# diwakar-vsingh/EKF-SLAM

Hardware: NVIDIA B200
Metric: filter-steps/s at N=100 features, batch 4096 filters (higher is better)
Workload: dtype f64

## Files before the change

### ekf-slam_b200/csrc/abi.cu

```cuda
#include <cmath>
#include <cstdio>
#include <cstdlib>
#include <cstring>
#include <climits>
#include <string>
#include <vector>

#include "common.cuh"

static thread_local std::string g_err;
extern "C" { static void step_graph_destroy(ekfslam_ctx* c); }

static int fail(int code, const std::string& msg) {
    g_err = msg;
    return code;
}

#define CK(call)                                                                              \
    do {                                                                                      \
        cudaError_t _e = (call);                                                              \
        if (_e != cudaSuccess)                                                                \
            return fail(EKFSLAM_ERR_CUDA, std::string(#call) + ": " + cudaGetErrorName(_e) + \
                                              " (" + cudaGetErrorString(_e) + ")");           \
    } while (0)

#define NEED_CTX(c)                                                     \
    do {                                                                \
        if (!(c)) return fail(EKFSLAM_ERR_INVALID, "null context");     \
        CK(cudaSetDevice((c)->device));                                 \
    } while (0)

struct KTimer {
    struct Rec { cudaEvent_t a, b; int slot; };
    std::vector<Rec> pending;
    std::vector<cudaEvent_t> pool;
    double ms[KT_COUNT];
    long long count[KT_COUNT];
    cudaEvent_t cur[KT_COUNT];
};

static cudaEvent_t kt_event(KTimer* t) {
    if (!t->pool.empty()) { cudaEvent_t e = t->pool.back(); t->pool.pop_back(); return e; }
    cudaEvent_t e = nullptr;
    if (cudaEventCreate(&e) != cudaSuccess) { cudaGetLastError(); return nullptr; }
    return e;
}

void kt_begin(ekfslam_ctx* c, int slot) {
    KTimer* t = c->timer;
    t->cur[slot] = kt_event(t);
    if (t->cur[slot]) cudaEventRecord(t->cur[slot], c->stream);
}

static void kt_drain_completed(KTimer* t) {
    size_t done = 0;
    while (done < t->pending.size() && cudaEventQuery(t->pending[done].b) == cudaSuccess) {
        KTimer::Rec& r = t->pending[done];
        float ms = 0.f;
        if (cudaEventElapsedTime(&ms, r.a, r.b) == cudaSuccess) { t->ms[r.slot] += ms; t->count[r.slot]++; }
        t->pool.push_back(r.a);
        t->pool.push_back(r.b);
        ++done;
    }
    cudaGetLastError();
    if (done) t->pending.erase(t->pending.begin(), t->pending.begin() + done);
}

void kt_end(ekfslam_ctx* c, int slot) {
    KTimer* t = c->timer;
    KTimer::Rec r;
    r.a = t->cur[slot]; r.b = r.a ? kt_event(t) : nullptr; r.slot = slot;
    if (!r.a || !r.b) { if (r.a) t->pool.push_back(r.a); return; }
    cudaEventRecord(r.b, c->stream);
    t->pending.push_back(r);
    if (t->pending.size() > 1024) kt_drain_completed(t);
}

static void kt_collect(ekfslam_ctx* c) {
    KTimer* t = c->timer;
    if (!t) return;
    for (auto& r : t->pending) {
        float ms = 0.f;
        if (cudaEventElapsedTime(&ms, r.a, r.b) == cudaSuccess) { t->ms[r.slot] += ms; t->count[r.slot]++; }
        t->pool.push_back(r.a);
        t->pool.push_back(r.b);
    }
    t->pending.clear();
}

static const char* KT_NAMES[KT_COUNT] = {"k_begin_frame", "k_predict", "k_features", "k_hp", "k_innov", "k_ransac",
                                         "k_upd_S", "k_chol", "k_w", "k_downdate_hi", "k_downdate", "k_symmetrize",
                                         "k_add_features", "k_wfix", "k_w_hi", "k_chol_hi", "k_upd_S_hi",
                                         "k_hp_rescue", "k_world", "k_eval", "k_cam_update", "k_downdate_cam"};

template <typename T>
static cudaError_t dalloc(T** p, size_t count, int64_t* total) {
    const size_t bytes = count * sizeof(T);
    cudaError_t e = cudaMalloc((void**)p, bytes ? bytes : 1);
    if (e == cudaSuccess) {
        *total += (int64_t)bytes;
        e = cudaMemset(*p, 0, bytes ? bytes : 1);
    }
    return e;
}

extern "C" {
// ... 104 lines not shown
    DA(v.S, Bz * v.N * 4);
    DA(v.z, Bz * v.N * 2);
    DA(v.zc, Bz * v.N * 2);
    DA(v.ftype, Bz * v.N);
    DA(v.flags, Bz * v.N);
    DA(v.mflags, Bz * v.N);
    DA(v.foff, Bz * v.N);
    DA(v.nstate, Bz);
    DA(v.nfeat, Bz);
    DA(v.counters, Bz * v.N * 2);
    DA(v.tag, Bz * v.N);
    DA(c->mm_del, Bz * v.N);
    DA(c->mm_quota, Bz);
    DA(c->det_n, Bz);
    DA(v.sel, Bz * v.N);
    DA(v.ksel, Bz);
    DA(v.stats, Bz);
    DA(v.nhyp_tab, (size_t)(v.N + 1) * (v.N + 2) / 2);
#undef DA
    ekfslam_camera cam;
    ekfslam_default_camera(&cam);
    set_devcam(c, &cam);
    ekfslam_default_params(&c->prm);
    std::vector<int32_t> tab;
    build_nhyp_table(tab, v.N, c->prm.p_spurious_free);
    cudaError_t e = cudaMemcpy(v.nhyp_tab, tab.data(), tab.size() * sizeof(int32_t), cudaMemcpyHostToDevice);
    if (e == cudaSuccess) e = cudaStreamCreateWithFlags(&c->own_stream, cudaStreamNonBlocking);
    if (e == cudaSuccess) e = cudaStreamCreateWithFlags(&c->copy_stream, cudaStreamNonBlocking);
    if (e == cudaSuccess) e = cudaStreamCreateWithFlags(&c->aux_stream, cudaStreamNonBlocking);
    if (e == cudaSuccess) e = cudaStreamCreateWithFlags(&c->aux2_stream, cudaStreamNonBlocking);
    if (e == cudaSuccess) e = cudaEventCreateWithFlags(&c->ev_join2, cudaEventDisableTiming);
    if (e == cudaSuccess) e = cudaEventCreateWithFlags(&c->ev_fork, cudaEventDisableTiming);
    if (e == cudaSuccess) e = cudaEventCreateWithFlags(&c->ev_join, cudaEventDisableTiming);
    if (e == cudaSuccess) e = cudaMallocHost((void**)&c->kmax_host, sizeof(int32_t));
    if (e == cudaSuccess) e = cudaEventCreateWithFlags(&c->ev_in, cudaEventDisableTiming);
    if (e == cudaSuccess) e = cudaEventCreateWithFlags(&c->ev_out, cudaEventDisableTiming);
    if (e == cudaSuccess) e = cudaEventCreateWithFlags(&c->ev_main, cudaEventDisableTiming);
    if (e != cudaSuccess) {
        ekfslam_destroy(c);
        return fail(EKFSLAM_ERR_CUDA, std::string("context init: ") + cudaGetErrorString(e));
    }
    c->stream = c->own_stream;
    cudaDeviceGetAttribute(&c->sm_count, cudaDevAttrMultiProcessorCount, device);
    if (c->sm_count <= 0) c->sm_count = 148;
    *out = c;
    return EKFSLAM_OK;
}

int ekfslam_destroy(ekfslam_ctx* c) {
    if (!c) return EKFSLAM_OK;
    cudaSetDevice(c->device);
    if (c->own_zc) { c->v.zc = c->own_zc; c->v.mflags = c->own_mflags; c->v.u = c->own_u; c->own_zc = nullptr; }
    DevView& v = c->v;
    void* ptrs[] = {v.x, v.xp, v.P, v.G, v.W, v.Sb, v.Li, v.yv, v.jn, v.jnt, v.ktot, v.kmaxdev, v.cv, v.h, v.Hc, v.S, v.z, v.zc, v.u, v.ftype,
                    v.flags, v.mflags, v.foff, v.nstate, v.nfeat, v.counters, v.tag, v.sel, v.ksel, v.stats, v.nhyp_tab,
                    c->mm_del, c->mm_quota, c->det_n, c->det_uv, c->det_tag, c->world_points, c->world_poses,
                    c->ev.rec, c->ev.tot, c->ev.ferr, c->ev.fnees, c->ev.mp, c->ev.mc,
                    c->cu.H, c->cu.z, c->cu.R, c->cu.on, c->cu.nis, c->cu.status};
    for (void* p : ptrs)
        if (p) cudaFree(p);
    if (c->timer) {
        cudaStreamSynchronize(c->stream);
        kt_collect(c);
        for (cudaEvent_t e : c->timer->pool) cudaEventDestroy(e);
        delete c->timer;
        c->timer = nullptr;
    }
    step_graph_destroy(c);
    if (c->own_stream) cudaStreamDestroy(c->own_stream);
    if (c->copy_stream) cudaStreamDestroy(c->copy_stream);
    if (c->aux_stream) cudaStreamDestroy(c->aux_stream);
    if (c->aux2_stream) cudaStreamDestroy(c->aux2_stream);
    if (c->ev_join2) cudaEventDestroy(c->ev_join2);
    if (c->ev_fork) cudaEventDestroy(c->ev_fork);
    if (c->ev_join) cudaEventDestroy(c->ev_join);
    if (c->ev_in) cudaEventDestroy(c->ev_in);
    if (c->ev_out) cudaEventDestroy(c->ev_out);
    if (c->ev_main) cudaEventDestroy(c->ev_main);
    if (c->pin) cudaFree(c->pin);
    if (c->kmax_host) cudaFreeHost(c->kmax_host);
    delete c;
    return EKFSLAM_OK;
}

int ekfslam_set_stream(ekfslam_ctx* c, void* s) {
    NEED_CTX(c);
    c->stream = s ? (cudaStream_t)s : c->own_stream;
    return EKFSLAM_OK;
}

int ekfslam_set_camera(ekfslam_ctx* c, const ekfslam_camera* cam) {
    NEED_CTX(c);
    if (!cam) return fail(EKFSLAM_ERR_INVALID, "cam is null");
    if (!(cam->dx > 0) || !(cam->dy > 0) || cam->nRows <= 0 || cam->nCols <= 0)
        return fail(EKFSLAM_ERR_INVALID, "camera: dx, dy, nRows, nCols must be positive");
    set_devcam(c, cam);
    return EKFSLAM_OK;
}

int ekfslam_set_params(ekfslam_ctx* c, const ekfslam_params* p) {
    NEED_CTX(c);
    if (!p) return fail(EKFSLAM_ERR_INVALID, "params is null");
    if (p->max_hyp <= 0 || p->fixed_hyp < 0 || !(p->p_spurious_free > 0 && p->p_spurious_free < 1))
        return fail(EKFSLAM_ERR_INVALID, "params: max_hyp > 0, fixed_hyp >= 0, 0 < p_spurious_free < 1");
    const bool retab = p->p_spurious_free != c->prm.p_spurious_free;
    c->prm = *p;
    if (retab) {
        std::vector<int32_t> tab;
// ... 314 lines not shown
    launch_innov(c, mode);
    LAUNCHED();
    return EKFSLAM_OK;
}

int ekfslam_gate(ekfslam_ctx* c) {
    NEED_CTX(c);
    return gate_mode(c, 1);
}

int ekfslam_apply_matches(ekfslam_ctx* c) {
    NEED_CTX(c);
    return gate_mode(c, 2);
}

int ekfslam_ransac(ekfslam_ctx* c) {
    NEED_CTX(c);
    if (c->v.n_u <= 0) return fail(EKFSLAM_ERR_STATE, "ransac: no uniform stream uploaded (ekfslam_upload_uniforms)");
    launch_ransac(c);
    LAUNCHED();
    return EKFSLAM_OK;
}

int ekfslam_update_masked(ekfslam_ctx* c, int mask, int which_prior) {
    NEED_CTX(c);
    if (!(mask & 0xff)) return fail(EKFSLAM_ERR_INVALID, "empty mask");
    launch_update(c, mask, which_prior ? 1 : 0);
    LAUNCHED();
    return EKFSLAM_OK;
}

int ekfslam_update_li(ekfslam_ctx* c) {
    NEED_CTX(c);
    launch_hp(c, EKFSLAM_F_HAS_H | EKFSLAM_F_LI, 0);
    return ekfslam_update_masked(c, EKFSLAM_F_LI, 1);
}

int ekfslam_update_iterated(ekfslam_ctx* c, int mask, int which_prior, int n_iter) {
    NEED_CTX(c);
    if (!(mask & 0xff)) return fail(EKFSLAM_ERR_INVALID, "empty mask");
    if (n_iter < 1 || n_iter > 64) return fail(EKFSLAM_ERR_INVALID, "n_iter must be in [1, 64]");
    DevView& v = c->v;
    const size_t xbytes = sizeof(double) * (size_t)v.B * v.ld;
    if (which_prior) CK(cudaMemcpyAsync(v.x, v.xp, xbytes, cudaMemcpyDeviceToDevice, c->stream));
    else CK(cudaMemcpyAsync(v.xp, v.x, xbytes, cudaMemcpyDeviceToDevice, c->stream));
    for (int j = 0; j < n_iter; ++j) {
        launch_features(c, 0, 3);
        launch_hp(c, mask & 0xff, 0);
        launch_update(c, mask, 1, 1 | (j + 1 < n_iter ? 2 : 0));
    }
    LAUNCHED();
    return EKFSLAM_OK;
}

int ekfslam_rescue(ekfslam_ctx* c) {
    NEED_CTX(c);
    launch_features(c, 0, 3);
    launch_innov_gather(c, 3);
    launch_hp(c, EKFSLAM_F_HAS_H | EKFSLAM_F_HI, 0, KT_HP_RESCUE);
    LAUNCHED();
    return EKFSLAM_OK;
}

int ekfslam_update_hi(ekfslam_ctx* c) { return ekfslam_update_masked(c, EKFSLAM_F_HI, 0); }

int ekfslam_step(ekfslam_ctx* c, int reset, int match_mode) {
    NEED_CTX(c);
    if (match_mode < 0 || match_mode > 2) return fail(EKFSLAM_ERR_INVALID, "match_mode must be 0, 1 or 2");
    if (c->v.n_u <= 0) return fail(EKFSLAM_ERR_STATE, "step: no uniform stream uploaded");
    if (reset) launch_begin_frame(c);
    launch_predict(c);
    launch_features(c, 1, 3);
    launch_innov_gather(c, 0);
    if (c->wait_inputs) { cudaStreamWaitEvent(c->stream, c->ev_in, 0); c->wait_inputs = 0; }
    if (match_mode) launch_innov(c, match_mode);
    launch_ransac(c);
    {
        if (c->prm.fixed_hyp <= 0) launch_hp(c, EKFSLAM_F_HAS_H | EKFSLAM_F_LI, 0);
        launch_update(c, EKFSLAM_F_LI, 1);
        launch_features(c, 0, 3);
        launch_innov_gather(c, 3);
        launch_hp(c, EKFSLAM_F_HAS_H | EKFSLAM_F_HI, 0, KT_HP_RESCUE);
        launch_update(c, EKFSLAM_F_HI, 0);
    }
    LAUNCHED();
    return EKFSLAM_OK;
}

struct StepGraph {
    cudaGraphExec_t exec;
    DevView v; ekfslam_params prm; DevCam cam;
    int reset, match_mode;
    int64_t launches;
};

static void step_graph_destroy(ekfslam_ctx* c) {
    StepGraph* g = (StepGraph*)c->step_graph;
    if (g) { if (g->exec) cudaGraphExecDestroy(g->exec); delete g; c->step_graph = nullptr; }
}

int ekfslam_step_graph(ekfslam_ctx* c, int reset, int match_mode) {
    NEED_CTX(c);
    DevView& v = c->v;
    if (c->timer || chol_lockstep(v) || c->wait_inputs || c->arm_out) return ekfslam_step(c, reset, match_mode);
    if (match_mode < 0 || match_mode > 2) return fail(EKFSLAM_ERR_INVALID, "match_mode must be 0, 1 or 2");
    if (v.n_u <= 0) return fail(EKFSLAM_ERR_STATE, "step: no uniform stream uploaded");
    StepGraph* g = (StepGraph*)c->step_graph;
    if (g && (memcmp(&g->v, &v, sizeof(DevView)) || memcmp(&g->prm, &c->prm, sizeof(ekfslam_params)) ||
              memcmp(&g->cam, &c->cam, sizeof(DevCam)) || g->reset != reset || g->match_mode != match_mode)) {
        step_graph_destroy(c);
        g = nullptr;
    }
    if (!g) {
        g = new (std::nothrow) StepGraph();
        if (!g) return fail(EKFSLAM_ERR_NOMEM, "host allocation failed");
        memset(g, 0, sizeof(*g));
// ... 455 lines not shown
```

### ekf-slam_b200/csrc/common.cuh

```cuda
#pragma once
#include <cuda_runtime.h>
#include <stdint.h>
#include <mutex>
#include "../../include/ekfslam.h"

#define EKF_XV 13
#define EKF_HC 13
#define EKF_HSTRIDE 26

struct DevCam {
    double k1, k2, Cx, Cy, f, dx, dy;
    double fku, fkv;
    double nRows, nCols;
};

struct DevView {
    int B, N, nmax, ld;
    int kmax;
    int n_u;
    double* x;
    double* xp;
    double* P;
    double* G;
    double* W;
// ... 49 lines not shown
    ekfslam_eval* rec;
    ekfslam_eval* tot;
    double* ferr;
    double* fnees;
    double* mp;
    double* mc;
};

struct DevCamUpd {
    double* H;
    double* z;
    double* R;
    uint8_t* on;
    double* nis;
    int32_t* status;
    int m, b0, nb;
    double gate;
};

struct ekfslam_ctx {
    int device;
    KTimer* timer;
    DevView v;
    DevCam cam;
    ekfslam_params prm;
    cudaStream_t own_stream;
    cudaStream_t stream;
    int64_t bytes;
    int64_t launches;
    int stage;
    cudaStream_t copy_stream;
    cudaStream_t aux_stream, aux2_stream;
    cudaEvent_t ev_fork, ev_join, ev_join2;
    cudaEvent_t ev_in, ev_out, ev_main;
    int wait_inputs;
    int arm_out;
    void* pin;
    size_t pin_bytes;
    int u_cap;
    void* step_graph;
    int sm_count;
    int32_t* kmax_host;
    DevWorld world;
    double* world_points; double* world_poses;
    double* det_uv; int32_t* det_tag; int32_t* det_n; int det_K;
    uint8_t* mm_del; int32_t* mm_quota;
    double* own_zc; uint8_t* own_mflags; double* own_u; int own_n_u;
    DevEval ev;
    DevCamUpd cu;
};

#define EKF_WPAD 68
__host__ __device__ __forceinline__ size_t w_at(int wrows, int t, int c) {
    return ((size_t)(c >> 6) * wrows + t) * EKF_WPAD + (c & 63);
}

__device__ __forceinline__ void w_fold_jt(double* w, const double* Jt) {
    const double w3 = w[0], w4 = w[1], w5 = w[2], w6 = w[3];
#pragma unroll
    for (int i = 0; i < 4; ++i) w[i] = w3 * Jt[i * 4 + 0] + w4 * Jt[i * 4 + 1] + w5 * Jt[i * 4 + 2] + w6 * Jt[i * 4 + 3];
}

#define EKF_TRI(nic, s) (((nic) * ((nic) + 1)) / 2 + (s))

inline bool chol_lockstep(const DevView& v) { return v.B < 128 && v.kmax >= 256; }

inline std::mutex& ekf_attr_mutex() { static std::mutex m; return m; }

void kt_begin(ekfslam_ctx* c, int slot);
void kt_end(ekfslam_ctx* c, int slot);
struct KScope {
    ekfslam_ctx* c; int slot;
    KScope(ekfslam_ctx* c_, int s_) : c(c_), slot(s_) { if (c->timer) kt_begin(c, slot); }
    ~KScope() { if (c->timer) kt_end(c, slot); c->launches++; }
};

#define ENSURE_DYN_SMEM(func, bytes, dev)                                                                    \
    do {                                                                                                     \
        static size_t _hw[64];                                                                               \
        const size_t _b = (size_t)(bytes);                                                                   \
        const int _d = (dev) & 63;                                                                           \
        if (_b > 48 * 1024) {                                                                                \
            std::lock_guard<std::mutex> _g(ekf_attr_mutex());    \
            if (_b > _hw[_d]) {                                                                              \
                cudaFuncSetAttribute(func, cudaFuncAttributeMaxDynamicSharedMemorySize, (int)_b);            \
                _hw[_d] = _b;                                                                                \
            }                                                                                                \
        }                                                                                                    \
    } while (0)

void launch_begin_frame(ekfslam_ctx* c);
void launch_predict(ekfslam_ctx* c);
void launch_features(ekfslam_ctx* c, int which, int parts);
void launch_hp(ekfslam_ctx* c, int need, int forbid, int slot = KT_HP);
void launch_innov_gather(ekfslam_ctx* c, int mode);
void launch_innov(ekfslam_ctx* c, int mode);
void launch_symmetrize(ekfslam_ctx* c, int b0, int nb);
void launch_ransac(ekfslam_ctx* c);
void launch_update(ekfslam_ctx* c, int mask, int which_prior, int flags = 0);
void launch_downdate(ekfslam_ctx* c, int slot);
void launch_chol_blocked64(ekfslam_ctx* c, int kact);
void launch_reset_filters(ekfslam_ctx* c, int b0, int nb, const double* d_xv, const double* d_Pxv);
void launch_id2cart(ekfslam_ctx* c, double threshold, int force_index, int32_t* d_conv);
void launch_delete_features(ekfslam_ctx* c, int b0, int nb, const uint8_t* d_del);
void launch_add_features(ekfslam_ctx* c, int b0, int nb, const double* d_uvd, int uvd_stride, const uint8_t* d_add,
                         const int32_t* d_quota, int j, const int32_t* d_tag, int tag_stride,
                         double std_pxl, double rho0, double std_rho);
void launch_world_candidates(ekfslam_ctx* c, int t);
void launch_world_detect(ekfslam_ctx* c, int t);
void launch_world_uniforms(ekfslam_ctx* c, int t);
void launch_mm_plan(ekfslam_ctx* c, int min_features);
void launch_eval(ekfslam_ctx* c, int mode, int t, int b0, int nb);
void launch_cam_update(ekfslam_ctx* c, int which);
```

### ekf-slam_b200/csrc/k_model.cu

```cuda
#include <cstdlib>
#include "model.cuh"
#include "tc_common.cuh"

__global__ void k_begin_frame(DevView v) {
    const int t = blockIdx.x * blockDim.x + threadIdx.x;
    if (t >= v.B * v.N) return;
    const int b = t / v.N, i = t - b * v.N;
    if (i >= v.nfeat[b]) return;
    const uint8_t f = v.flags[t];
    if (f & EKFSLAM_F_HAS_H) v.counters[2 * t] += 1;
    if (f & (EKFSLAM_F_LI | EKFSLAM_F_HI)) v.counters[2 * t + 1] += 1;
    v.flags[t] = f & EKFSLAM_F_CAND;
}

void launch_begin_frame(ekfslam_ctx* c) {
    const int tot = c->v.B * c->v.N;
    KScope ks(c, KT_BEGIN_FRAME);
    k_begin_frame<<<(tot + 255) / 256, 256, 0, c->stream>>>(c->v);
}

__global__ void __launch_bounds__(256, 3) k_predict(DevView v, ekfslam_params prm) {
    const int b = blockIdx.x;
    const int n = v.nstate[b];
    const int ld = v.ld;
// ... 280 lines not shown
            for (int r = 0; r < 7; ++r) {
                g0.x += Hs[r] * pc[r].x; g0.y += Hs[r] * pc[r].y;
                g1.x += Hs[EKF_HC + r] * pc[r].x; g1.y += Hs[EKF_HC + r] * pc[r].y;
            }
            const int off = sOff[s];
            const int w = sW[s];
            const double* Pr = P + (size_t)off * ld + c0;
            if (w == 6) {
                double2 pf[6];
#pragma unroll
                for (int r = 0; r < 6; ++r) pf[r] = *reinterpret_cast<const double2*>(Pr + (size_t)r * ld);
#pragma unroll
                for (int r = 0; r < 6; ++r) {
                    g0.x += Hs[7 + r] * pf[r].x; g0.y += Hs[7 + r] * pf[r].y;
                    g1.x += Hs[EKF_HC + 7 + r] * pf[r].x; g1.y += Hs[EKF_HC + 7 + r] * pf[r].y;
                }
            } else {
                double2 pf[3];
#pragma unroll
                for (int r = 0; r < 3; ++r) pf[r] = *reinterpret_cast<const double2*>(Pr + (size_t)r * ld);
#pragma unroll
                for (int r = 0; r < 3; ++r) {
                    g0.x += Hs[7 + r] * pf[r].x; g0.y += Hs[7 + r] * pf[r].y;
                    g1.x += Hs[EKF_HC + 7 + r] * pf[r].x; g1.y += Hs[EKF_HC + 7 + r] * pf[r].y;
                }
            }
            const int i = sIdx[s];
            *reinterpret_cast<double2*>(G + (size_t)(2 * i) * ld + c0) = g0;
            *reinterpret_cast<double2*>(G + (size_t)(2 * i + 1) * ld + c0) = g1;
        }
    }
}

void launch_hp(ekfslam_ctx* c, int need, int forbid, int slot) {
    const int colchunks = (c->v.nmax + 255) / 256;
    const long long base = (long long)colchunks * c->v.B;
    const long long want = 4LL * c->sm_count;
    int fch = HP_CHUNK;
    while (fch > 8 && base * ((c->v.N + fch - 1) / fch) < want) fch >>= 1;
    int fz = (c->v.N + fch - 1) / fch;
    if (base >= want) fz = 1;
    else if (base * fz > want) fz = (int)((want + base - 1) / base);
    dim3 grid(colchunks, c->v.B, fz);
    KScope ks(c, slot);
    k_hp<<<grid, 128, 0, c->stream>>>(c->v, need, forbid, fch);
}

__global__ void __launch_bounds__(128) k_innov(DevView v, ekfslam_params prm, int mode) {
    const int t = blockIdx.x * blockDim.x + threadIdx.x;
    if (t >= v.B * v.N) return;
    const int b = t / v.N, i = t - b * v.N;
    if (i >= v.nfeat[b]) return;
    if (v.ftype[t] == EKFSLAM_FEAT_NONE) return;
    const uint8_t f = v.flags[t];
    if (mode == 2) {
        const uint8_t m = v.mflags[t] & (EKFSLAM_F_HAS_Z | EKFSLAM_F_IC);
        if (m) {
            v.z[2 * t] = v.zc[2 * t]; v.z[2 * t + 1] = v.zc[2 * t + 1];
            v.flags[t] = f | m;
        }
        return;
    }
    if (!(f & EKFSLAM_F_HAS_H) || !(v.mflags[t] & EKFSLAM_F_CAND)) return;
    const double s00 = v.S[4 * t], s01 = v.S[4 * t + 1], s10 = v.S[4 * t + 2], s11 = v.S[4 * t + 3];
    const double zu = v.zc[2 * t], zv = v.zc[2 * t + 1];
    const double n0 = zu - v.h[2 * t], n1 = zv - v.h[2 * t + 1];
    const double det = s00 * s11 - s01 * s10;
    const double d2 = (n0 * (s11 * n0 - s01 * n1) + n1 * (-s10 * n0 + s00 * n1)) / det;
    const double tr = s00 + s11;
    const double disc = sqrt((s00 - s11) * (s00 - s11) + 4.0 * s01 * s10);
    const double lmax = 0.5 * (tr + disc);
    if (lmax < 100.0 && d2 < prm.chi2_gate) {
        v.z[2 * t] = zu; v.z[2 * t + 1] = zv;
        v.flags[t] = f | EKFSLAM_F_HAS_Z | EKFSLAM_F_IC;
    }
}

#ifndef IG_MINB
// ... 442 lines not shown
```

### ekf-slam_b200/csrc/k_update.cu

```cuda
#include "model.cuh"
#include "tc_common.cuh"

#define NB 16

__device__ __forceinline__ void tri_unrank(int e, int& r, int& c) {
    r = (int)((sqrt(8.0 * e + 1.0) - 1.0) * 0.5);
    while ((r + 1) * (r + 2) / 2 <= e) ++r;
    while (r * (r + 1) / 2 > e) --r;
    c = e - r * (r + 1) / 2;
}

#define UPS_NMAX 128
template <bool STAGED>
__device__ __forceinline__ void upd_S_pairs(const DevView& v, int b, int ns, int first, int stride, const int* s_sel,
                                            const int* s_off, const int* s_w, const double* s_H) {
    const int N = v.N, ld = v.ld, kmax = v.kmax;
    const int* __restrict__ sel = v.sel + (size_t)b * N;
    const double* __restrict__ G = v.G + (size_t)b * kmax * ld;
    double* __restrict__ S = v.Sb + (size_t)b * kmax * kmax;
    const int npair = ns * (ns + 1) / 2;
    for (int e = first; e < npair; e += stride) {
        int fa, fb;
        tri_unrank(e, fa, fb);
        int ia, off, w;
        const double* __restrict__ H;
        if (STAGED) {
            ia = s_sel[fa]; off = s_off[fb]; w = s_w[fb]; H = s_H + fb * EKF_HSTRIDE;
        } else {
            ia = sel[fa];
            const size_t tb = (size_t)b * N + sel[fb];
            H = v.Hc + tb * EKF_HSTRIDE;
            off = v.foff[tb];
            w = (v.ftype[tb] == EKFSLAM_FEAT_INVERSEDEPTH) ? 6 : 3;
        }
        const double* __restrict__ g0 = G + (size_t)(2 * ia) * ld;
        const double* __restrict__ g1 = g0 + ld;
        double ga[EKF_HC], gb[EKF_HC];
#pragma unroll
        for (int c = 0; c < 7; ++c) { ga[c] = g0[c]; gb[c] = g1[c]; }
#pragma unroll
        for (int c = 0; c < 6; ++c) {
            const int cc = off + ((c < w) ? c : 0);
            ga[7 + c] = g0[cc]; gb[7 + c] = g1[cc];
        }
        double s00 = 0, s01 = 0, s10 = 0, s11 = 0;
#pragma unroll
        for (int c = 0; c < EKF_HC; ++c) {
            if (c < 7 + w) {
                const double h0 = H[c], h1 = H[EKF_HC + c];
                s00 += ga[c] * h0; s01 += ga[c] * h1; s10 += gb[c] * h0; s11 += gb[c] * h1;
            }
        }
        if (fa == fb) { s00 += 1.0; s11 += 1.0; }
        S[(size_t)(2 * fa) * kmax + 2 * fb] = s00;
        S[(size_t)(2 * fa) * kmax + 2 * fb + 1] = s01;
        S[(size_t)(2 * fa + 1) * kmax + 2 * fb] = s10;
        S[(size_t)(2 * fa + 1) * kmax + 2 * fb + 1] = s11;
    }
}

__global__ void __launch_bounds__(256, 4) k_upd_S(DevView v, int mask, int which_prior, int iter_nu, int do_pairs) {
    const int b = blockIdx.x;
    const int N = v.N, ld = v.ld, kmax = v.kmax;
    const int nf = v.nfeat[b];
    const int tid = threadIdx.x;
    __shared__ int s_k;
    int* __restrict__ sel = v.sel + (size_t)b * N;
    if (tid < 32) {
        int cnt = 0;
        for (int i0 = 0; i0 < nf; i0 += 32) {
            const int i = i0 + tid;
            const bool on = (i < nf) && v.ftype[b * N + i] != EKFSLAM_FEAT_NONE && (v.flags[(size_t)b * N + i] & mask);
            const unsigned m = __ballot_sync(0xffffffffu, on);
            if (on) sel[cnt + __popc(m & ((1u << tid) - 1u))] = i;
            cnt += __popc(m);
        }
        if (tid == 0) {
            v.ksel[b] = cnt;
            s_k = cnt;
            if (mask & EKFSLAM_F_LI) v.stats[b].n_li = cnt;
            if (mask & EKFSLAM_F_HI) v.stats[b].n_hi = cnt;
            if (cnt > 0) atomicMax(v.kmaxdev, 2 * cnt);
        }
    }
    __syncthreads();
    const int ns = s_k;
    const int k = 2 * ns;
    {
        double* __restrict__ yv0 = v.yv + (size_t)b * kmax;
        const double* __restrict__ xj = v.x + (size_t)b * ld;
        const double* __restrict__ x0 = v.xp + (size_t)b * ld;
        for (int a = tid; a < k; a += blockDim.x) {
            const size_t t = (size_t)b * N + sel[a >> 1];
            double nu = v.z[2 * t + (a & 1)] - v.h[2 * t + (a & 1)];
            if (iter_nu) {
                const double* __restrict__ H = v.Hc + t * EKF_HSTRIDE + (a & 1) * EKF_HC;
                const int off = v.foff[t];
                const int w = (v.ftype[t] == EKFSLAM_FEAT_INVERSEDEPTH) ? 6 : 3;
                double s = 0.0;
                for (int c = 0; c < 7; ++c) s += H[c] * (x0[c] - xj[c]);
                for (int c = 0; c < w; ++c) s += H[7 + c] * (x0[off + c] - xj[off + c]);
                nu -= s;
            }
            yv0[a] = nu;
        }
    }
    __syncthreads();
    if (which_prior == 1) {
        const int n = v.nstate[b];
        for (int j = tid; j < n; j += blockDim.x) v.x[(size_t)b * ld + j] = v.xp[(size_t)b * ld + j];
    }
    if (k == 0) return;
    if (!do_pairs) return;
    if (N <= UPS_NMAX) {
        __shared__ int s_sel[UPS_NMAX], s_off[UPS_NMAX], s_w[UPS_NMAX];
        __shared__ double s_H[UPS_NMAX * EKF_HSTRIDE];
        for (int f = tid; f < ns; f += blockDim.x) {
            const int i = sel[f];
            const size_t t = (size_t)b * N + i;
            s_sel[f] = i;
            s_off[f] = v.foff[t];
            s_w[f] = (v.ftype[t] == EKFSLAM_FEAT_INVERSEDEPTH) ? 6 : 3;
        }
        for (int e = tid; e < ns * EKF_HSTRIDE; e += blockDim.x) {
            const int f = e / EKF_HSTRIDE;
            s_H[e] = v.Hc[((size_t)b * N + sel[f]) * EKF_HSTRIDE + (e - f * EKF_HSTRIDE)];
        }
        __syncthreads();
        upd_S_pairs<true>(v, b, ns, tid, blockDim.x, s_sel, s_off, s_w, s_H);
    } else {
        upd_S_pairs<false>(v, b, ns, tid, blockDim.x, nullptr, nullptr, nullptr, nullptr);
    }
}

__global__ void __launch_bounds__(256) k_upd_pairs(DevView v) {
    const int b = blockIdx.y;
    const int ns = v.ksel[b];
    if (ns == 0) return;
    upd_S_pairs<false>(v, b, ns, blockIdx.x * blockDim.x + threadIdx.x, gridDim.x * blockDim.x, nullptr, nullptr, nullptr, nullptr);
}

__global__ void __launch_bounds__(128) k_chol(DevView v, int kskip) {
    extern __shared__ double sm[];
    const int b = blockIdx.x;
    const int k = 2 * v.ksel[b];
    if (k == 0 || k <= kskip) return;
    const int kmax = v.kmax;
    const int tid = threadIdx.x, lane = tid & 31, warp = tid >> 5;
    double* __restrict__ S = v.Sb + (size_t)b * kmax * kmax;
    double* __restrict__ X = v.Li + (size_t)b * kmax * kmax;
    double* D = sm;
    double* Di = D + NB * (NB + 1);
    double* Pn = Di + NB * (NB + 1);
    __shared__ int s_bad;
    if (tid == 0) s_bad = 0;

    for (int j0 = 0; j0 < k; j0 += NB) {
        const int nb = min(NB, k - j0);
        for (int e = tid; e < NB * NB; e += blockDim.x) {
            const int r = e / NB, c = e - r * NB;
            D[r * (NB + 1) + c] = (r < nb && c <= r) ? S[(size_t)(j0 + r) * kmax + j0 + c] : ((r >= nb && r == c) ? 1.0 : 0.0);
            Di[r * (NB + 1) + c] = 0.0;
        }
        __syncthreads();
        if (warp == 0) {
            if (chol16_warp(D, NB + 1, Di) && lane == 0) s_bad = 1;
        }
        __syncthreads();
        for (int e = tid; e < nb * nb; e += blockDim.x) {
            const int r = e / nb, c = e - r * nb;
            if (c <= r) {
                S[(size_t)(j0 + r) * kmax + j0 + c] = D[r * (NB + 1) + c];
// ... 736 lines not shown
#pragma unroll
        for (int a = 0; a < KW; ++a) {
            if (a < k) {
                double sacc = 0.0;
#pragma unroll
                for (int t = 0; t <= a; ++t) sacc += Xs[a][t] * g[t];
                wcol[(size_t)a * EKF_WPAD] = incol ? sacc : 0.0;
            }
        }
        if (incol) x[c] += xs;
    }
    if (finalize) {
        __syncthreads();
        if (tid == 0) normjac_normalize(x, v.jnt + (size_t)b * 16);
    }
}

__global__ void __launch_bounds__(128) k_wfix(DevView v) {
    const int b = blockIdx.x;
    const int k = 2 * v.ksel[b];
    double* __restrict__ W = v.W + (size_t)b * v.wstride;
    __shared__ double Jt[16];
    if (threadIdx.x < 16) Jt[threadIdx.x] = v.jnt[(size_t)b * 16 + threadIdx.x];
    __syncthreads();
    for (int a = threadIdx.x; a < k; a += blockDim.x) w_fold_jt(W + w_at(v.wrows, a, 3), Jt);
    if (threadIdx.x < 16 && k > 0) v.jn[(size_t)b * 16 + threadIdx.x] = Jt[threadIdx.x];
    if (threadIdx.x == 0) v.ktot[b] = k;
}

static void gemm_attr(ekfslam_ctx* c, size_t w_sm) {
    ENSURE_DYN_SMEM(k_gemm<0>, w_sm, c->device);
}

void launch_update(ekfslam_ctx* c, int mask, int which_prior, int flags) {
    DevView& v = c->v;
    cudaStream_t st = c->stream;
    const bool hi = (mask & EKFSLAM_F_HI) != 0;
    cudaMemsetAsync(v.kmaxdev, 0, sizeof(int32_t), st);
    {
        KScope ks(c, hi ? KT_UPD_S_HI : KT_UPD_S);
        const int slices = (v.B < 296) ? (int)((8 * 148 + v.B - 1) / v.B) : 1;
        k_upd_S<<<v.B, 256, 0, st>>>(v, mask, which_prior, flags & 1, slices == 1);
        if (slices > 1) { dim3 gp(slices, v.B); k_upd_pairs<<<gp, 256, 0, st>>>(v); c->launches++; }
    }
    const size_t chol_sm = sizeof(double) * (2 * NB * (NB + 1) + (size_t)v.kmax * (NB + 1));
    const size_t chs_sm = CHS_SMEM(CHS_K);
    const size_t chss_sm = CHS_SMEM(CHS_KS);
    ENSURE_DYN_SMEM(k_chol, chol_sm, c->device);
    const size_t chsm_sm = CHS_SMEM(CHS_KM);
    ENSURE_DYN_SMEM((k_chol_sm<CHS_KM, 256, 0, 3>), chsm_sm, c->device);
    ENSURE_DYN_SMEM((k_chol_sm<CHS_K, 256, CHS_KM, 2>), chs_sm, c->device);
    ENSURE_DYN_SMEM((k_chol_sm<CHS_K, 256, 0, 2>), chs_sm, c->device);
    ENSURE_DYN_SMEM((k_chol_sm<CHS_K, 256, CHS_KS, 2>), chs_sm, c->device);
    ENSURE_DYN_SMEM((k_chol_sm<CHS_KM, 256, CHS_KS, 3>), chsm_sm, c->device);
    const size_t chl_sm = CHS_SMEM(CHS_KL);
    ENSURE_DYN_SMEM((k_chol_sm<CHS_KL, 512, CHS_K, 1>), chl_sm, c->device);
    if (chol_lockstep(v)) {
        launch_chol_lockstep(c);
    } else {
        KScope ks(c, hi ? KT_CHOL_HI : KT_CHOL);
        const bool use_mid = v.kmax > CHS_KM;
        const bool large = use_mid && v.kmax > CHS_K;
        auto fork_large = [&]() {
            if (!large) return;
            cudaStreamWaitEvent(c->aux2_stream, c->ev_fork, 0);
            k_chol_sm<CHS_KL, 512, CHS_K, 1><<<v.B, 512, chl_sm, c->aux2_stream>>>(v);
            cudaEventRecord(c->ev_join2, c->aux2_stream);
            c->launches++;
        };
        auto join_large = [&]() { if (large) cudaStreamWaitEvent(st, c->ev_join2, 0); };
        if (hi) {
            if (use_mid) {
                cudaEventRecord(c->ev_fork, st);
                cudaStreamWaitEvent(c->aux_stream, c->ev_fork, 0);
                cudaStreamWaitEvent(c->aux2_stream, c->ev_fork, 0);
                k_chol_w32<<<(v.B + 3) / 4, 128, 0, c->aux_stream>>>(v);
                k_chol_sm<CHS_K, 256, CHS_KM, 2><<<v.B, 256, chs_sm, c->aux_stream>>>(v);
                cudaEventRecord(c->ev_join, c->aux_stream);
                k_chol_sm<CHS_KS, 128, CHW_K><<<v.B, 128, chss_sm, c->aux2_stream>>>(v);
                if (large) { k_chol_sm<CHS_KL, 512, CHS_K, 1><<<v.B, 512, chl_sm, c->aux2_stream>>>(v); c->launches++; }
                cudaEventRecord(c->ev_join2, c->aux2_stream);
                k_chol_sm<CHS_KM, 256, CHS_KS, 3><<<v.B, 256, chsm_sm, st>>>(v);
                cudaStreamWaitEvent(st, c->ev_join, 0);
                cudaStreamWaitEvent(st, c->ev_join2, 0);
                c->launches += 3;
            } else {
                k_chol_w32<<<(v.B + 3) / 4, 128, 0, st>>>(v);
                k_chol_sm<CHS_KS, 128, CHW_K><<<v.B, 128, chss_sm, st>>>(v);
                k_chol_sm<CHS_K, 256, CHS_KS, 2><<<v.B, 256, chs_sm, st>>>(v);
                c->launches += 2;
            }
        } else {
            if (use_mid) {
                cudaEventRecord(c->ev_fork, st);
                cudaStreamWaitEvent(c->aux_stream, c->ev_fork, 0);
                k_chol_sm<CHS_K, 256, CHS_KM, 2><<<v.B, 256, chs_sm, c->aux_stream>>>(v);
                cudaEventRecord(c->ev_join, c->aux_stream);
                fork_large();
                k_chol_sm<CHS_KM, 256, 0, 3><<<v.B, 256, chsm_sm, st>>>(v);
                cudaStreamWaitEvent(st, c->ev_join, 0);
                join_large();
                c->launches++;
            } else {
                k_chol_sm<CHS_K, 256, 0, 2><<<v.B, 256, chs_sm, st>>>(v);
            }
        }
        const int kres = large ? CHS_KL : CHS_K;
        if (v.kmax > kres) { k_chol<<<v.B, 128, chol_sm, st>>>(v, kres); c->launches++; }
    }
    int cg = hi ? 2 : 1;
    {
        const long long ctas = (long long)((v.kmax + TM - 1) / TM) * v.B;
        const int want = (int)((8LL * 148 + ctas - 1) / ctas);
        const int ncb_max = (v.nmax + TM - 1) / TM;
        if (want > cg) cg = want < ncb_max ? want : ncb_max;
    }
    dim3 gw((v.kmax + TM - 1) / TM, cg, v.B);
    const size_t w_sm = sizeof(double) * (NSTAGE * (TM * APAD + TK * TPAD) + v.kmax + 256) + sizeof(int) * v.kmax;
    gemm_attr(c, w_sm);
    {
        KScope ks(c, hi ? KT_W_HI : KT_W);
        const int fin = (flags & 2) ? 0 : 1;
        const size_t ws_sm = sizeof(double) * 2 * WS_K * 128;
        ENSURE_DYN_SMEM((k_w_small<WS_K, 0, 3>), ws_sm, c->device);
        k_w_small<WS_K, 0, 3><<<v.B, 128, ws_sm, st>>>(v, fin);
        c->launches++;
        k_gemm<0><<<gw, 256, w_sm, st>>>(v, fin, WS_K);
    }
    if (flags & 2) return;
    { KScope ks(c, KT_WFIX); k_wfix<<<v.B, 128, 0, st>>>(v); }
    if (c->arm_out && (mask & EKFSLAM_F_HI)) { cudaEventRecord(c->ev_out, st); c->arm_out = 0; }
    launch_downdate(c, (mask & EKFSLAM_F_HI) ? KT_DOWNDATE_HI : KT_DOWNDATE);
}
```

Baseline: 249,100.

## Compute innovation covariance directly from P and overlap HP on side stream

k_upd_S now builds S = H P H^T + R per feature pair straight from P, instead of reading the precomputed G = H P. It stages each feature's H, P cross-blocks and camera projections in dynamic shared memory. The HP kernel launch moves inside launch_update, so it runs on a dedicated stream concurrently with the Cholesky factorisation and is joined before the W gemm. This removes HP from the critical path before S and Cholesky, at the cost of more shared memory per block, lower occupancy (launch bounds 4 reduced to 2), and extra stream/event bookkeeping.

```diff
diff --git a/ekf-slam_b200/csrc/abi.cu b/ekf-slam_b200/csrc/abi.cu
--- a/ekf-slam_b200/csrc/abi.cu
+++ b/ekf-slam_b200/csrc/abi.cu
@@ -46,10 +46,10 @@
     return e;
 }
 
-void kt_begin(ekfslam_ctx* c, int slot) {
+void kt_begin(ekfslam_ctx* c, int slot, cudaStream_t st) {
     KTimer* t = c->timer;
     t->cur[slot] = kt_event(t);
-    if (t->cur[slot]) cudaEventRecord(t->cur[slot], c->stream);
+    if (t->cur[slot]) cudaEventRecord(t->cur[slot], st);
 }
 
 static void kt_drain_completed(KTimer* t) {
@@ -66,12 +66,12 @@
     if (done) t->pending.erase(t->pending.begin(), t->pending.begin() + done);
 }
 
-void kt_end(ekfslam_ctx* c, int slot) {
+void kt_end(ekfslam_ctx* c, int slot, cudaStream_t st) {
     KTimer* t = c->timer;
     KTimer::Rec r;
     r.a = t->cur[slot]; r.b = r.a ? kt_event(t) : nullptr; r.slot = slot;
     if (!r.a || !r.b) { if (r.a) t->pool.push_back(r.a); return; }
-    cudaEventRecord(r.b, c->stream);
+    cudaEventRecord(r.b, st);
     t->pending.push_back(r);
     if (t->pending.size() > 1024) kt_drain_completed(t);
 }
@@ -242,6 +242,8 @@
     if (e == cudaSuccess) e = cudaEventCreateWithFlags(&c->ev_join2, cudaEventDisableTiming);
     if (e == cudaSuccess) e = cudaEventCreateWithFlags(&c->ev_fork, cudaEventDisableTiming);
     if (e == cudaSuccess) e = cudaEventCreateWithFlags(&c->ev_join, cudaEventDisableTiming);
+    if (e == cudaSuccess) e = cudaStreamCreateWithFlags(&c->hp_stream, cudaStreamNonBlocking);
+    if (e == cudaSuccess) e = cudaEventCreateWithFlags(&c->ev_hp, cudaEventDisableTiming);
     if (e == cudaSuccess) e = cudaMallocHost((void**)&c->kmax_host, sizeof(int32_t));
     if (e == cudaSuccess) e = cudaEventCreateWithFlags(&c->ev_in, cudaEventDisableTiming);
     if (e == cudaSuccess) e = cudaEventCreateWithFlags(&c->ev_out, cudaEventDisableTiming);
@@ -284,6 +286,8 @@
     if (c->ev_join2) cudaEventDestroy(c->ev_join2);
     if (c->ev_fork) cudaEventDestroy(c->ev_fork);
     if (c->ev_join) cudaEventDestroy(c->ev_join);
+    if (c->hp_stream) cudaStreamDestroy(c->hp_stream);
+    if (c->ev_hp) cudaEventDestroy(c->ev_hp);
     if (c->ev_in) cudaEventDestroy(c->ev_in);
     if (c->ev_out) cudaEventDestroy(c->ev_out);
     if (c->ev_main) cudaEventDestroy(c->ev_main);
@@ -664,8 +668,9 @@
 
 int ekfslam_update_li(ekfslam_ctx* c) {
     NEED_CTX(c);
-    launch_hp(c, EKFSLAM_F_HAS_H | EKFSLAM_F_LI, 0);
-    return ekfslam_update_masked(c, EKFSLAM_F_LI, 1);
+    launch_update(c, EKFSLAM_F_LI, 1, 0, EKFSLAM_F_HAS_H | EKFSLAM_F_LI);
+    LAUNCHED();
+    return EKFSLAM_OK;
 }
 
 int ekfslam_update_iterated(ekfslam_ctx* c, int mask, int which_prior, int n_iter) {
@@ -678,8 +683,7 @@
     else CK(cudaMemcpyAsync(v.xp, v.x, xbytes, cudaMemcpyDeviceToDevice, c->stream));
     for (int j = 0; j < n_iter; ++j) {
         launch_features(c, 0, 3);
-        launch_hp(c, mask & 0xff, 0);
-        launch_update(c, mask, 1, 1 | (j + 1 < n_iter ? 2 : 0));
+        launch_update(c, mask, 1, 1 | (j + 1 < n_iter ? 2 : 0), mask & 0xff);
     }
     LAUNCHED();
     return EKFSLAM_OK;
@@ -708,12 +712,10 @@
     if (match_mode) launch_innov(c, match_mode);
     launch_ransac(c);
     {
-        if (c->prm.fixed_hyp <= 0) launch_hp(c, EKFSLAM_F_HAS_H | EKFSLAM_F_LI, 0);
-        launch_update(c, EKFSLAM_F_LI, 1);
+        launch_update(c, EKFSLAM_F_LI, 1, 0, c->prm.fixed_hyp <= 0 ? EKFSLAM_F_HAS_H | EKFSLAM_F_LI : 0);
         launch_features(c, 0, 3);
         launch_innov_gather(c, 3);
-        launch_hp(c, EKFSLAM_F_HAS_H | EKFSLAM_F_HI, 0, KT_HP_RESCUE);
-        launch_update(c, EKFSLAM_F_HI, 0);
+        launch_update(c, EKFSLAM_F_HI, 0, 0, EKFSLAM_F_HAS_H | EKFSLAM_F_HI, KT_HP_RESCUE);
     }
     LAUNCHED();
     return EKFSLAM_OK;
diff --git a/ekf-slam_b200/csrc/common.cuh b/ekf-slam_b200/csrc/common.cuh
--- a/ekf-slam_b200/csrc/common.cuh
+++ b/ekf-slam_b200/csrc/common.cuh
@@ -105,6 +105,8 @@
     cudaStream_t copy_stream;
     cudaStream_t aux_stream, aux2_stream;
     cudaEvent_t ev_fork, ev_join, ev_join2;
+    cudaStream_t hp_stream;
+    cudaEvent_t ev_hp;
     cudaEvent_t ev_in, ev_out, ev_main;
     int wait_inputs;
     int arm_out;
@@ -140,12 +142,13 @@
 
 inline std::mutex& ekf_attr_mutex() { static std::mutex m; return m; }
 
-void kt_begin(ekfslam_ctx* c, int slot);
-void kt_end(ekfslam_ctx* c, int slot);
+void kt_begin(ekfslam_ctx* c, int slot, cudaStream_t st);
+void kt_end(ekfslam_ctx* c, int slot, cudaStream_t st);
 struct KScope {
-    ekfslam_ctx* c; int slot;
-    KScope(ekfslam_ctx* c_, int s_) : c(c_), slot(s_) { if (c->timer) kt_begin(c, slot); }
-    ~KScope() { if (c->timer) kt_end(c, slot); c->launches++; }
+    ekfslam_ctx* c; int slot; cudaStream_t st;
+    KScope(ekfslam_ctx* c_, int s_) : KScope(c_, s_, c_->stream) {}
+    KScope(ekfslam_ctx* c_, int s_, cudaStream_t st_) : c(c_), slot(s_), st(st_) { if (c->timer) kt_begin(c, slot, st); }
+    ~KScope() { if (c->timer) kt_end(c, slot, st); c->launches++; }
 };
 
 #define ENSURE_DYN_SMEM(func, bytes, dev)                                                                    \
@@ -165,12 +168,12 @@
 void launch_begin_frame(ekfslam_ctx* c);
 void launch_predict(ekfslam_ctx* c);
 void launch_features(ekfslam_ctx* c, int which, int parts);
-void launch_hp(ekfslam_ctx* c, int need, int forbid, int slot = KT_HP);
+void launch_hp(ekfslam_ctx* c, int need, int forbid, int slot = KT_HP, cudaStream_t st = nullptr);
 void launch_innov_gather(ekfslam_ctx* c, int mode);
 void launch_innov(ekfslam_ctx* c, int mode);
 void launch_symmetrize(ekfslam_ctx* c, int b0, int nb);
 void launch_ransac(ekfslam_ctx* c);
-void launch_update(ekfslam_ctx* c, int mask, int which_prior, int flags = 0);
+void launch_update(ekfslam_ctx* c, int mask, int which_prior, int flags = 0, int hp_need = 0, int hp_slot = KT_HP);
 void launch_downdate(ekfslam_ctx* c, int slot);
 void launch_chol_blocked64(ekfslam_ctx* c, int kact);
 void launch_reset_filters(ekfslam_ctx* c, int b0, int nb, const double* d_xv, const double* d_Pxv);
diff --git a/ekf-slam_b200/csrc/k_model.cu b/ekf-slam_b200/csrc/k_model.cu
--- a/ekf-slam_b200/csrc/k_model.cu
+++ b/ekf-slam_b200/csrc/k_model.cu
@@ -336,7 +336,8 @@
     }
 }
 
-void launch_hp(ekfslam_ctx* c, int need, int forbid, int slot) {
+void launch_hp(ekfslam_ctx* c, int need, int forbid, int slot, cudaStream_t st) {
+    if (!st) st = c->stream;
     const int colchunks = (c->v.nmax + 255) / 256;
     const long long base = (long long)colchunks * c->v.B;
     const long long want = 4LL * c->sm_count;
@@ -346,8 +347,8 @@
     if (base >= want) fz = 1;
     else if (base * fz > want) fz = (int)((want + base - 1) / base);
     dim3 grid(colchunks, c->v.B, fz);
-    KScope ks(c, slot);
-    k_hp<<<grid, 128, 0, c->stream>>>(c->v, need, forbid, fch);
+    KScope ks(c, slot, st);
+    k_hp<<<grid, 128, 0, st>>>(c->v, need, forbid, fch);
 }
 
 __global__ void __launch_bounds__(128) k_innov(DevView v, ekfslam_params prm, int mode) {
diff --git a/ekf-slam_b200/csrc/k_update.cu b/ekf-slam_b200/csrc/k_update.cu
--- a/ekf-slam_b200/csrc/k_update.cu
+++ b/ekf-slam_b200/csrc/k_update.cu
@@ -10,56 +10,120 @@
     c = e - r * (r + 1) / 2;
 }
 
+__device__ __forceinline__ void g_cam(const double* __restrict__ Ha, int wa, const double* __restrict__ Pc, int ldc,
+                                      const double* __restrict__ Aa, int lda, int row, int c, double& g) {
+    const double* __restrict__ h = Ha + row * EKF_HC;
+    double s = 0.0;
+#pragma unroll
+    for (int r = 0; r < 7; ++r) s += h[r] * Pc[r * ldc + c];
+#pragma unroll
+    for (int r = 0; r < 6; ++r)
+        if (r < wa) s += h[7 + r] * Aa[r * lda + c];
+    g = s;
+}
+__device__ __forceinline__ void s_pair(const double* __restrict__ Ha, int wa, const double* __restrict__ gca,
+                                       const double* __restrict__ Hb, int wb, const double* __restrict__ Ab, int ldb,
+                                       const double* __restrict__ Pab, int ld, bool diag, double (&s)[4]) {
+    double pb[6][6];
+    const bool odd = ((size_t)Pab >> 3) & 1;
+#pragma unroll
+    for (int r = 0; r < 6; ++r) {
+#pragma unroll
+        for (int j = 0; j < 6; ++j) pb[r][j] = 0.0;
+        if (r < wa) {
+            const double* __restrict__ p = Pab + (size_t)r * ld;
+            if (wb == 6) {
+                if (odd) {
+                    pb[r][0] = p[0];
+                    const double2 d1 = *reinterpret_cast<const double2*>(p + 1), d3 = *reinterpret_cast<const double2*>(p + 3);
+                    pb[r][1] = d1.x; pb[r][2] = d1.y; pb[r][3] = d3.x; pb[r][4] = d3.y;
+                    pb[r][5] = p[5];
+                } else {
+                    const double2 d0 = *reinterpret_cast<const double2*>(p), d2 = *reinterpret_cast<const double2*>(p + 2),
+                                  d4 = *reinterpret_cast<const double2*>(p + 4);
+                    pb[r][0] = d0.x; pb[r][1] = d0.y; pb[r][2] = d2.x; pb[r][3] = d2.y; pb[r][4] = d4.x; pb[r][5] = d4.y;
+                }
+            } else {
+                if (odd) {
+                    pb[r][0] = p[0];
+                    const double2 d1 = *reinterpret_cast<const double2*>(p + 1);
+                    pb[r][1] = d1.x; pb[r][2] = d1.y;
+                } else {
+                    const double2 d0 = *reinterpret_cast<const double2*>(p);
+                    pb[r][0] = d0.x; pb[r][1] = d0.y; pb[r][2] = p[2];
+                }
+            }
+        }
+    }
+    double s00 = 0.0, s01 = 0.0, s10 = 0.0, s11 = 0.0;
+#pragma unroll
+    for (int c = 0; c < 7; ++c) {
+        const double ga = gca[c], gb = gca[7 + c], h0 = Hb[c], h1 = Hb[EKF_HC + c];
+        s00 += ga * h0; s01 += ga * h1; s10 += gb * h0; s11 += gb * h1;
+    }
+#pragma unroll
+    for (int j = 0; j < 6; ++j) {
+        if (j < wb) {
+            double ga = 0.0, gb = 0.0;
+#pragma unroll
+            for (int r = 0; r < 7; ++r) {
+                const double pv = Ab[j * ldb + r];
+                ga += Ha[r] * pv; gb += Ha[EKF_HC + r] * pv;
+            }
+#pragma unroll
+            for (int r = 0; r < 6; ++r)
+                if (r < wa) { ga += Ha[7 + r] * pb[r][j]; gb += Ha[EKF_HC + 7 + r] * pb[r][j]; }
+            const double h0 = Hb[7 + j], h1 = Hb[EKF_HC + 7 + j];
+            s00 += ga * h0; s01 += ga * h1; s10 += gb * h0; s11 += gb * h1;
+        }
+    }
+    if (diag) { s00 += 1.0; s11 += 1.0; }
+    s[0] = s00; s[1] = s01; s[2] = s10; s[3] = s11;
+}
+
 #define UPS_NMAX 128
+#define UPS_PC 50
+#define UPS_F 82
+#define UPS_SMEM(N) (sizeof(double) * (UPS_PC + (size_t)(N) * UPS_F) + sizeof(int) * 2 * (size_t)(N))
 template <bool STAGED>
-__device__ __forceinline__ void upd_S_pairs(const DevView& v, int b, int ns, int first, int stride, const int* s_sel,
-                                            const int* s_off, const int* s_w, const double* s_H) {
+__device__ __forceinline__ void upd_S_pairs(const DevView& v, int b, int ns, int first, int stride, const int* s_off,
+                                            const int* s_w, const double* s_st) {
     const int N = v.N, ld = v.ld, kmax = v.kmax;
     const int* __restrict__ sel = v.sel + (size_t)b * N;
-    const double* __restrict__ G = v.G + (size_t)b * kmax * ld;
+    const double* __restrict__ P = v.P + (size_t)b * v.nmax * ld;
     double* __restrict__ S = v.Sb + (size_t)b * kmax * kmax;
     const int npair = ns * (ns + 1) / 2;
     for (int e = first; e < npair; e += stride) {
         int fa, fb;
         tri_unrank(e, fa, fb);
-        int ia, off, w;
-        const double* __restrict__ H;
+        double s[4];
         if (STAGED) {
-            ia = s_sel[fa]; off = s_off[fb]; w = s_w[fb]; H = s_H + fb * EKF_HSTRIDE;
+            const double* fa_st = s_st + UPS_PC + fa * UPS_F;
+            const double* fb_st = s_st + UPS_PC + fb * UPS_F;
+            s_pair(fa_st, s_w[fa], fa_st + 68, fb_st, s_w[fb], fb_st + 26, 7, P + (size_t)s_off[fa] * ld + s_off[fb], ld,
+                   fa == fb, s);
         } else {
-            ia = sel[fa];
-            const size_t tb = (size_t)b * N + sel[fb];
-            H = v.Hc + tb * EKF_HSTRIDE;
-            off = v.foff[tb];
-            w = (v.ftype[tb] == EKFSLAM_FEAT_INVERSEDEPTH) ? 6 : 3;
-        }
-        const double* __restrict__ g0 = G + (size_t)(2 * ia) * ld;
-        const double* __restrict__ g1 = g0 + ld;
-        double ga[EKF_HC], gb[EKF_HC];
-#pragma unroll
-        for (int c = 0; c < 7; ++c) { ga[c] = g0[c]; gb[c] = g1[c]; }
-#pragma unroll
-        for (int c = 0; c < 6; ++c) {
-            const int cc = off + ((c < w) ? c : 0);
-            ga[7 + c] = g0[cc]; gb[7 + c] = g1[cc];
-        }
-        double s00 = 0, s01 = 0, s10 = 0, s11 = 0;
-#pragma unroll
-        for (int c = 0; c < EKF_HC; ++c) {
-            if (c < 7 + w) {
-                const double h0 = H[c], h1 = H[EKF_HC + c];
-                s00 += ga[c] * h0; s01 += ga[c] * h1; s10 += gb[c] * h0; s11 += gb[c] * h1;
-            }
-        }
-        if (fa == fb) { s00 += 1.0; s11 += 1.0; }
-        S[(size_t)(2 * fa) * kmax + 2 * fb] = s00;
-        S[(size_t)(2 * fa) * kmax + 2 * fb + 1] = s01;
-        S[(size_t)(2 * fa + 1) * kmax + 2 * fb] = s10;
-        S[(size_t)(2 * fa + 1) * kmax + 2 * fb + 1] = s11;
-    }
-}
-
-__global__ void __launch_bounds__(256, 4) k_upd_S(DevView v, int mask, int which_prior, int iter_nu, int do_pairs) {
+            const size_t ta = (size_t)b * N + sel[fa], tb = (size_t)b * N + sel[fb];
+            const double* __restrict__ Ha = v.Hc + ta * EKF_HSTRIDE;
+            const int offa = v.foff[ta], offb = v.foff[tb];
+            const int wa = (v.ftype[ta] == EKFSLAM_FEAT_INVERSEDEPTH) ? 6 : 3;
+            const int wb = (v.ftype[tb] == EKFSLAM_FEAT_INVERSEDEPTH) ? 6 : 3;
+            double gca[14];
+#pragma unroll
+            for (int row = 0; row < 2; ++row)
+#pragma unroll
+                for (int cc = 0; cc < 7; ++cc) g_cam(Ha, wa, P, ld, P + (size_t)offa * ld, ld, row, cc, gca[row * 7 + cc]);
+            s_pair(Ha, wa, gca, v.Hc + tb * EKF_HSTRIDE, wb, P + (size_t)offb * ld, ld, P + (size_t)offa * ld + offb, ld,
+                   fa == fb, s);
+        }
+        S[(size_t)(2 * fa) * kmax + 2 * fb] = s[0];
+        S[(size_t)(2 * fa) * kmax + 2 * fb + 1] = s[1];
+        S[(size_t)(2 * fa + 1) * kmax + 2 * fb] = s[2];
+        S[(size_t)(2 * fa + 1) * kmax + 2 * fb + 1] = s[3];
+    }
+}
+
+__global__ void __launch_bounds__(256, 2) k_upd_S(DevView v, int mask, int which_prior, int iter_nu, int do_pairs) {
     const int b = blockIdx.x;
     const int N = v.N, ld = v.ld, kmax = v.kmax;
     const int nf = v.nfeat[b];
@@ -112,32 +176,42 @@
     }
     if (k == 0) return;
     if (!do_pairs) return;
-    if (N <= UPS_NMAX) {
-        __shared__ int s_sel[UPS_NMAX], s_off[UPS_NMAX], s_w[UPS_NMAX];
-        __shared__ double s_H[UPS_NMAX * EKF_HSTRIDE];
-        for (int f = tid; f < ns; f += blockDim.x) {
-            const int i = sel[f];
-            const size_t t = (size_t)b * N + i;
-            s_sel[f] = i;
-            s_off[f] = v.foff[t];
-            s_w[f] = (v.ftype[t] == EKFSLAM_FEAT_INVERSEDEPTH) ? 6 : 3;
-        }
-        for (int e = tid; e < ns * EKF_HSTRIDE; e += blockDim.x) {
-            const int f = e / EKF_HSTRIDE;
-            s_H[e] = v.Hc[((size_t)b * N + sel[f]) * EKF_HSTRIDE + (e - f * EKF_HSTRIDE)];
-        }
-        __syncthreads();
-        upd_S_pairs<true>(v, b, ns, tid, blockDim.x, s_sel, s_off, s_w, s_H);
-    } else {
-        upd_S_pairs<false>(v, b, ns, tid, blockDim.x, nullptr, nullptr, nullptr, nullptr);
-    }
+    extern __shared__ __align__(16) double ups[];
+    const double* __restrict__ P = v.P + (size_t)b * v.nmax * ld;
+    int* s_off = reinterpret_cast<int*>(ups + UPS_PC + (size_t)N * UPS_F);
+    int* s_w = s_off + N;
+    for (int f = tid; f < ns; f += blockDim.x) {
+        const size_t t = (size_t)b * N + sel[f];
+        s_off[f] = v.foff[t];
+        s_w[f] = (v.ftype[t] == EKFSLAM_FEAT_INVERSEDEPTH) ? 6 : 3;
+    }
+    if (tid < 49) ups[tid] = P[(size_t)(tid / 7) * ld + tid % 7];
+    for (int e = tid; e < ns * EKF_HSTRIDE; e += blockDim.x) {
+        const int f = e / EKF_HSTRIDE;
+        ups[UPS_PC + f * UPS_F + (e - f * EKF_HSTRIDE)] = v.Hc[((size_t)b * N + sel[f]) * EKF_HSTRIDE + (e - f * EKF_HSTRIDE)];
+    }
+    __syncthreads();
+    for (int e = tid; e < ns * 42; e += blockDim.x) {
+        const int f = e / 42, q = e - f * 42, r = q / 7;
+        ups[UPS_PC + f * UPS_F + EKF_HSTRIDE + q] = (r < s_w[f]) ? P[(size_t)(s_off[f] + r) * ld + (q - r * 7)] : 0.0;
+    }
+    __syncthreads();
+    for (int e = tid; e < ns * 14; e += blockDim.x) {
+        const int f = e / 14, q = e - f * 14;
+        const double* fs = ups + UPS_PC + f * UPS_F;
+        double g;
+        g_cam(fs, s_w[f], ups, 7, fs + EKF_HSTRIDE, 7, q / 7, q % 7, g);
+        ups[UPS_PC + f * UPS_F + 68 + q] = g;
+    }
+    __syncthreads();
+    upd_S_pairs<true>(v, b, ns, tid, blockDim.x, s_off, s_w, ups);
 }
 
 __global__ void __launch_bounds__(256) k_upd_pairs(DevView v) {
     const int b = blockIdx.y;
     const int ns = v.ksel[b];
     if (ns == 0) return;
-    upd_S_pairs<false>(v, b, ns, blockIdx.x * blockDim.x + threadIdx.x, gridDim.x * blockDim.x, nullptr, nullptr, nullptr, nullptr);
+    upd_S_pairs<false>(v, b, ns, blockIdx.x * blockDim.x + threadIdx.x, gridDim.x * blockDim.x, nullptr, nullptr, nullptr);
 }
 
 __global__ void __launch_bounds__(128) k_chol(DevView v, int kskip) {
@@ -940,7 +1014,7 @@
     ENSURE_DYN_SMEM(k_gemm<0>, w_sm, c->device);
 }
 
-void launch_update(ekfslam_ctx* c, int mask, int which_prior, int flags) {
+void launch_update(ekfslam_ctx* c, int mask, int which_prior, int flags, int hp_need, int hp_slot) {
     DevView& v = c->v;
     cudaStream_t st = c->stream;
     const bool hi = (mask & EKFSLAM_F_HI) != 0;
@@ -948,8 +1022,20 @@
     {
         KScope ks(c, hi ? KT_UPD_S_HI : KT_UPD_S);
         const int slices = (v.B < 296) ? (int)((8 * 148 + v.B - 1) / v.B) : 1;
-        k_upd_S<<<v.B, 256, 0, st>>>(v, mask, which_prior, flags & 1, slices == 1);
-        if (slices > 1) { dim3 gp(slices, v.B); k_upd_pairs<<<gp, 256, 0, st>>>(v); c->launches++; }
+        const bool staged = slices == 1 && v.N <= UPS_NMAX;
+        const size_t ups_sm = staged ? UPS_SMEM(v.N) : 0;
+        ENSURE_DYN_SMEM(k_upd_S, ups_sm, c->device);
+        k_upd_S<<<v.B, 256, ups_sm, st>>>(v, mask, which_prior, flags & 1, staged);
+        if (!staged) { dim3 gp(slices, v.B); k_upd_pairs<<<gp, 256, 0, st>>>(v); c->launches++; }
+    }
+    const bool hp_side = hp_need && !chol_lockstep(v);
+    if (hp_side) {
+        cudaEventRecord(c->ev_fork, st);
+        cudaStreamWaitEvent(c->hp_stream, c->ev_fork, 0);
+        launch_hp(c, hp_need, 0, hp_slot, c->hp_stream);
+        cudaEventRecord(c->ev_hp, c->hp_stream);
+    } else if (hp_need) {
+        launch_hp(c, hp_need, 0, hp_slot);
     }
     const size_t chol_sm = sizeof(double) * (2 * NB * (NB + 1) + (size_t)v.kmax * (NB + 1));
     const size_t chs_sm = CHS_SMEM(CHS_K);
@@ -1016,6 +1102,7 @@
         const int kres = large ? CHS_KL : CHS_K;
         if (v.kmax > kres) { k_chol<<<v.B, 128, chol_sm, st>>>(v, kres); c->launches++; }
     }
+    if (hp_side) cudaStreamWaitEvent(st, c->ev_hp, 0);
     int cg = hi ? 2 : 1;
     {
         const long long ctas = (long long)((v.kmax + TM - 1) / TM) * v.B;
```

Measured after the change: 237,500 (median of 6 runs). -4.7%, worse.
